# esrice/trio_binning

Hardware: AMD Instinct MI355X
Metric: Gbases/sec classified (k=21, 2x300M k-mer tables) (higher is better)
Workload: dtype u64

## Files before the change

include/tbk.h:

```cpp
#ifndef TBK_H
#define TBK_H

#include <stddef.h>
#include <stdint.h>

#ifdef __cplusplus
extern "C" {
#endif

#define TBK_ABI_VERSION 1

typedef enum tbk_status {
    TBK_OK = 0,
    TBK_ERR_INVALID = -1,
    TBK_ERR_IO = -2,
    TBK_ERR_FORMAT = -3,
    TBK_ERR_NO_DEVICE = -4,
    TBK_ERR_HIP = -5,
    TBK_ERR_NOMEM = -6,
    TBK_ERR_STATE = -7
} tbk_status;

typedef struct tbk_table tbk_table;
typedef struct tbk_classifier tbk_classifier;
// ... 39 lines not shown
    int32_t short_keys, entries, wide_entries, front;
    int32_t mod_sampling;
    int32_t span3;
    int32_t guests;
    int32_t minimizer_w;
    int32_t minimizer_m;
    int32_t two_read_kernel;
    double table_load;
    double entry_load, wentry_load, short_load;
    double clustered, behind_front, plainly_clustered, entry_min_ratio;
    uint64_t memory_budget_bytes;
    uint64_t table_align;
    uint32_t short_line_cap;
    int32_t probe_max_blocks;
    int32_t packed_h2d;
    uint64_t slice_bases;
    int32_t build_timing;
    int32_t force_replica;
    int32_t ring_streams, copy_priority, h2d_streams, zero_copy;
    int32_t full_keys;
    double full_load;
    int32_t replica_copy;
    int32_t verify_build;
} tbk_options;
void tbk_options_init(tbk_options *o);
int tbk_options_from_env(tbk_options *o);
int tbk_classifier_create_opts(const tbk_table *hap_a, const tbk_table *hap_b, const tbk_options *options, tbk_classifier **out);
int tbk_classifier_create_multi(const tbk_table *hap_a, const tbk_table *hap_b, const int *devices, int n_devices,
                                tbk_classifier **out );
int tbk_classifier_create_multi_opts(const tbk_table *hap_a, const tbk_table *hap_b, const int *devices, int n_devices,
                                     const tbk_options *options, tbk_classifier **out );
int tbk_classifier_replicate(const tbk_classifier *src, int device, tbk_classifier **out);
int tbk_classifier_table_id(const tbk_classifier *c, uint64_t *table_id, int *is_replica);
int tbk_classifier_device(const tbk_classifier *c);
int tbk_classifier_stats(const tbk_classifier *c, uint64_t *distinct_a, uint64_t *distinct_b,
                         uint64_t *n_buckets, uint64_t *table_bytes);
int tbk_classifier_shared_keys(const tbk_classifier *c, uint64_t *n_shared);
int tbk_classifier_layout(const tbk_classifier *c, int *minimizer_w, int *minimizer_m, int *span_offset);
int tbk_classifier_sampling_t(const tbk_classifier *c);
int tbk_classifier_build_info(const tbk_classifier *c, int *layout_builds, uint64_t *keys_past_half);
int tbk_classifier_front(const tbk_classifier *c, int *front, uint64_t *keys_behind_front);
int tbk_classifier_entries(const tbk_classifier *c, int *entry_layout, uint64_t *entries_a, uint64_t *entries_b);
int tbk_classifier_calibrate(tbk_classifier *c, double *lines_per_sec);
int tbk_classifier_calibrate_pairs(tbk_classifier *c, int inflight, int waves_per_simd, uint64_t n_lines, double *lines_per_sec);

int tbk_classify_batch(tbk_classifier *c, const uint8_t *bases, const uint64_t *offsets,
// ... 161 lines not shown
```

trio_binning_amd/_lib.py:

```python
import ctypes as C
import os

_HERE = os.path.dirname(os.path.abspath(__file__))
_NAME = "libtbk_hip.so"

TBK_OK = 0
TBK_ERR_INVALID = -1
TBK_ERR_IO = -2
TBK_ERR_FORMAT = -3
TBK_ERR_NO_DEVICE = -4
TBK_ERR_HIP = -5
TBK_ERR_NOMEM = -6
TBK_ERR_STATE = -7


class TbkError(RuntimeError):
    def __init__(self, code, message):
        super().__init__(f"libtbk_hip: {message} (status {code})")
        self.code = code
        self.message = message


def _find():
    override = os.environ.get("TBK_LIBRARY")
# ... 172 lines not shown
        _sig("tbk_fastx_inflates_on_device", C.c_int, _vp)
    if hasattr(lib, "tbk_bgzf_inflate_device"):
        _sig("tbk_bgzf_inflate_device", C.c_int, C.c_int, C.c_char_p, _u64, C.c_char_p, _u64, _u64p)
    if hasattr(lib, "tbk_bgzf_bench_device"):
        _sig("tbk_bgzf_bench_device", C.c_int, C.c_int, C.c_char_p, _u64, C.c_int, C.POINTER(C.c_double), C.POINTER(C.c_double), _u64p)
    if hasattr(lib, "tbk_gzip_bench_device"):
        _sig("tbk_gzip_bench_device", C.c_int, C.c_int, _vp, _u64p, _u64, C.c_int, C.POINTER(C.c_double), C.POINTER(C.c_double), _u64p)
_sig("tbk_gzip_member", C.c_int, C.c_char_p, C.c_size_t, C.c_char_p, C.c_size_t, C.POINTER(C.c_size_t))
_sig("tbk_crc32_c", C.c_uint32, C.c_uint32, C.c_char_p, C.c_size_t)
_sig("tbk_format_tsv", C.c_int, _vp, C.c_char_p, _vp, _vp, _vp, C.c_size_t, C.POINTER(C.c_size_t))
_sig("tbk_format_float", C.c_int, C.c_double, C.c_char_p, C.c_size_t)


class tbk_options(C.Structure):
    _fields_ = [("size", C.c_uint32),
                ("short_keys", C.c_int32), ("entries", C.c_int32), ("wide_entries", C.c_int32), ("front", C.c_int32),
                ("mod_sampling", C.c_int32), ("span3", C.c_int32), ("guests", C.c_int32), ("minimizer_w", C.c_int32), ("minimizer_m", C.c_int32),
                ("two_read_kernel", C.c_int32),
                ("table_load", C.c_double), ("entry_load", C.c_double), ("wentry_load", C.c_double), ("short_load", C.c_double),
                ("clustered", C.c_double), ("behind_front", C.c_double), ("plainly_clustered", C.c_double), ("entry_min_ratio", C.c_double),
                ("memory_budget_bytes", C.c_uint64), ("table_align", C.c_uint64), ("short_line_cap", C.c_uint32), ("probe_max_blocks", C.c_int32),
                ("packed_h2d", C.c_int32), ("slice_bases", C.c_uint64), ("build_timing", C.c_int32), ("force_replica", C.c_int32),
                ("ring_streams", C.c_int32), ("copy_priority", C.c_int32), ("h2d_streams", C.c_int32), ("zero_copy", C.c_int32),
                ("full_keys", C.c_int32), ("full_load", C.c_double), ("replica_copy", C.c_int32), ("verify_build", C.c_int32)]


HAS_OPTIONS = hasattr(lib, "tbk_classifier_create_opts")
if HAS_OPTIONS:
    _sig("tbk_options_init", None, C.POINTER(tbk_options))
    _sig("tbk_options_from_env", C.c_int, C.POINTER(tbk_options))
    _sig("tbk_classifier_create_opts", C.c_int, _vp, _vp, C.POINTER(tbk_options), C.POINTER(_vp))
    _sig("tbk_classifier_create_multi_opts", C.c_int, _vp, _vp, C.POINTER(C.c_int), C.c_int, C.POINTER(tbk_options), C.POINTER(_vp))
    _sig("tbk_pipeline_create_opts", C.c_int, _vp, _vp, C.POINTER(C.c_int), C.c_int, C.POINTER(tbk_options), C.POINTER(_vp))


def last_error() -> str:
    msg = lib.tbk_last_error()
    return msg.decode("utf-8", "replace") if msg else ""


def check(status: int) -> None:
    if status == TBK_OK:
        return
    msg = last_error()
    if status == TBK_ERR_IO:
        raise IOError(msg)
    if status in (TBK_ERR_FORMAT, TBK_ERR_INVALID):
# ... 45 lines not shown
```

trio_binning_amd/csrc/tbk_common.h:

```cpp
#pragma once
#include <stdint.h>
#include "tbk_tmer_order.h"

#ifdef __HIPCC__
#define TBK_HD __host__ __device__ __forceinline__
#else
#define TBK_HD inline
#endif

#define TBK_EMPTY 0xFFFFFFFFFFFFFFFFull
#define TBK_NOKEY 0xFFFFFFFFFFFFFFFEull
#define TBK_SLOTS_PER_BUCKET 8
#define TBK_BUCKET_BYTES 64
#define TBK_GUEST 0x8000000000000000ull

struct TbkMz {
    int w;
    int m;
    int o;
    int t;
};

TBK_HD uint32_t tbk_mix32(uint64_t key) {
    uint32_t lo = (uint32_t)key, hi = (uint32_t)(key >> 32);
    uint32_t h = lo * 0x9E3779B1u ^ (hi + 0x7F4A7C15u) * 0x85EBCA77u;
    h ^= h >> 15;
    h *= 0xC2B2AE3Du;
    h ^= h >> 13;
    return h;
}

TBK_HD uint32_t tbk_reduce(uint32_t h, uint32_t n_buckets) {
    return (uint32_t)(((uint64_t)h * (uint64_t)n_buckets) >> 32);
}
// ... 548 lines not shown
```

trio_binning_amd/csrc/tbk_host.cpp:

```cpp
#include <hip/hip_runtime.h>

#include <fcntl.h>
#include <sys/mman.h>
#include <sys/stat.h>
#include <unistd.h>

#include <algorithm>
#include <chrono>
#include <cmath>
#include <cerrno>
#include <cstdarg>
#include <cstdio>
#include <cstdlib>
#include <cstring>
#include <cctype>
#include <pthread.h>
#include <sched.h>
#include <atomic>
#include <memory>
#include <mutex>
#include <string>
#include <thread>
#include <vector>

#include "../../include/tbk.h"
#include "tbk_common.h"
#include "tbk_pack.h"

extern "C" hipError_t tbk_launch_order(uint64_t *, uint64_t, const uint32_t *, const uint32_t *, uint32_t, uint32_t, hipStream_t);
extern "C" hipError_t tbk_launch_insert(uint64_t *, uint32_t, uint32_t, uint32_t, TbkMz, const uint64_t *, uint64_t, uint32_t *, uint32_t *, uint32_t, TbkTableView,
                                        unsigned long long *, unsigned long long *, int *, hipStream_t);
extern "C" hipError_t tbk_launch_contains(TbkTableView, const uint64_t *, uint64_t, uint8_t *, hipStream_t);
extern "C" hipError_t tbk_launch_entry_insert(uint64_t *, uint32_t, uint32_t, TbkMz, int, const uint64_t *, uint64_t, int, int, unsigned long long *, int *, hipStream_t);
extern "C" hipError_t tbk_launch_short_insert(uint64_t *, uint32_t, uint32_t, uint32_t, TbkMz, int, const uint64_t *, uint64_t, int, unsigned long long *, int *, uint32_t, hipStream_t);
extern "C" hipError_t tbk_launch_full_insert(uint64_t *, uint32_t, uint32_t, TbkMz, int, const uint64_t *, uint64_t, int, unsigned long long *, int *, uint32_t, hipStream_t);
extern "C" hipError_t tbk_launch_probe_index(const uint64_t *, uint64_t, uint64_t, int32_t *, uint32_t *, uint64_t, int, hipStream_t);
extern "C" int tbk_probe_has_two_read_kernel(TbkMz);
extern "C" hipError_t tbk_launch_probe_range(const uint8_t *, const uint32_t *, const uint16_t *, const uint64_t *, uint64_t, uint64_t, TbkPairView, int,
                                             int32_t *, uint32_t *, uint64_t, uint64_t, uint64_t, int, int, hipEvent_t, hipStream_t, int);
extern "C" hipError_t tbk_launch_scatter_bad(const uint32_t *, const uint16_t *, uint64_t, uint16_t *, uint64_t, int, hipStream_t);
extern "C" uint64_t tbk_packed_chunks(uint64_t total_bases);
extern "C" uint64_t tbk_probe_passes(uint64_t total);
static constexpr uint64_t TBK_PASS_BASES = 2048;
extern "C" hipError_t tbk_launch_synth_keys(uint64_t, uint64_t, uint64_t, int, uint64_t *, hipStream_t);
extern "C" hipError_t tbk_launch_synth_reads(uint64_t, uint64_t, uint64_t, uint32_t, uint64_t, uint64_t, uint64_t,
                                             int, int, int, uint8_t *, uint64_t *, hipStream_t);
extern "C" hipError_t tbk_launch_fill(void *, uint64_t, uint64_t, hipStream_t);
extern "C" hipError_t tbk_launch_stream(const void *, uint64_t, uint32_t *, hipStream_t);
extern "C" hipError_t tbk_launch_gather(const void *, uint64_t, int, int, int, uint64_t, uint64_t, uint32_t *,
                                        uint64_t *, hipStream_t);

static thread_local std::string g_err;

static int fail(int code, const char *fmt, ...) {
    char buf[512];
    va_list ap;
    va_start(ap, fmt);
    vsnprintf(buf, sizeof buf, fmt, ap);
    va_end(ap);
    g_err = buf;
    return code;
}
// ... 27 lines not shown
    return end == v ? dflt : d;
}

extern "C" void tbk_options_init(tbk_options *o) {
    if (!o) return;
    memset(o, 0, sizeof *o);
    o->size = (uint32_t)sizeof *o;
    o->short_keys = o->entries = o->wide_entries = o->front = -1;
    o->full_keys = -1;
    o->full_load = 2.0;
    o->mod_sampling = o->span3 = o->guests = -1;
    o->minimizer_w = -1;
    o->minimizer_m = 0;
    o->two_read_kernel = 1;
    o->table_load = 0.0;
    o->entry_load = 0.5; o->wentry_load = 0.25; o->short_load = 2.3;
    o->clustered = 0.003; o->behind_front = 0.05; o->plainly_clustered = 0.12; o->entry_min_ratio = 1.5;
    o->memory_budget_bytes = 0;
    o->short_line_cap = 32;
    o->packed_h2d = 1;
    o->slice_bases = (uint64_t)384 << 20;
    o->h2d_streams = 1;
    o->verify_build = -1;
}

extern "C" int tbk_options_from_env(tbk_options *o) {
    if (!o) return fail(TBK_ERR_INVALID, "options is NULL");
    if (o->size != sizeof *o) tbk_options_init(o);
    auto tri = [](const char *name, int32_t &v) { const double d = env_double(name, -1); if (getenv(name) && *getenv(name)) v = d > 0 ? 1 : d == 0 ? 0 : -1; };
    auto num = [](const char *name, double &v) { if (getenv(name) && *getenv(name)) v = env_double(name, v); };
    auto inum = [](const char *name, int32_t &v) { if (getenv(name) && *getenv(name)) v = (int32_t)env_double(name, v); };
    auto unum = [](const char *name, uint64_t &v) { if (getenv(name) && *getenv(name)) v = (uint64_t)std::max(0.0, env_double(name, (double)v)); };
    tri("TBK_SHORT", o->short_keys); tri("TBK_ENTRY", o->entries); tri("TBK_ENTRY_WIDE", o->wide_entries); tri("TBK_FRONT", o->front);
    tri("TBK_FULL", o->full_keys); num("TBK_FULL_LOAD", o->full_load);
    tri("TBK_MOD_SAMPLING", o->mod_sampling); tri("TBK_SPAN3", o->span3); tri("TBK_GUESTS", o->guests);
    inum("TBK_MINIMIZER_W", o->minimizer_w); inum("TBK_MINIMIZER_M", o->minimizer_m); inum("TBK_TWO_READ", o->two_read_kernel);
    num("TBK_TABLE_LOAD", o->table_load); num("TBK_ENTRY_LOAD", o->entry_load); num("TBK_WENTRY_LOAD", o->wentry_load); num("TBK_SHORT_LOAD", o->short_load);
    num("TBK_CLUSTERED", o->clustered); num("TBK_BEHIND_FRONT", o->behind_front); num("TBK_PLAINLY_CLUSTERED", o->plainly_clustered);
    num("TBK_ENTRY_MIN_RATIO", o->entry_min_ratio);
    unum("TBK_MEMORY_BUDGET", o->memory_budget_bytes); unum("TBK_TABLE_ALIGN", o->table_align); unum("TBK_SLICE_BASES", o->slice_bases);
    { uint64_t cap = o->short_line_cap; unum("TBK_SHORT_LINE_CAP", cap); o->short_line_cap = (uint32_t)cap; }
    inum("TBK_PROBE_MAX_BLOCKS", o->probe_max_blocks); inum("TBK_PACKED_H2D", o->packed_h2d); inum("TBK_BUILD_TIMING", o->build_timing);
    inum("TBK_FORCE_REPLICA", o->force_replica); inum("TBK_RING_STREAMS", o->ring_streams); inum("TBK_COPY_PRIORITY", o->copy_priority);
    inum("TBK_H2D_STREAMS", o->h2d_streams); inum("TBK_ZERO_COPY", o->zero_copy);
    inum("TBK_REPLICA_COPY", o->replica_copy); tri("TBK_VERIFY_BUILD", o->verify_build);
    return TBK_OK;
}

static tbk_options resolve_options(const tbk_options *in) {
    tbk_options o;
    tbk_options_init(&o);
    if (in && in->size >= 8) memcpy(&o, in, std::min<size_t>(in->size, sizeof o));
    o.size = (uint32_t)sizeof o;
    return o;
}

static long local_ranks() {
    long ranks = (long)env_double("TBK_LOCAL_RANKS", 0);
    if (ranks < 1) ranks = (long)env_double("LOCAL_WORLD_SIZE", 1);
    return std::max<long>(1, ranks);
}

static long usable_cpus() {
    long n = (long)std::thread::hardware_concurrency();
    if (n < 1) n = 1;
    cpu_set_t set;
    if (sched_getaffinity(0, sizeof set, &set) == 0 && CPU_COUNT(&set) > 0) n = std::min<long>(n, CPU_COUNT(&set));
// ... 1733 lines not shown
    }
    delete c;
}

static void par_memcpy(void *dst, const void *src, size_t n) {
    const size_t piece = (size_t)16 << 20;
    const int nt = (int)std::min<size_t>((size_t)tbk_host_threads(), n / piece);
    if (nt <= 1) { memcpy(dst, src, n); return; }
    std::vector<std::thread> pool;
    for (int t = 0; t < nt; t++) {
        const size_t lo = n * (size_t)t / nt, hi = n * (size_t)(t + 1) / nt;
        pool.emplace_back([=]() { memcpy((char *)dst + lo, (const char *)src + lo, hi - lo); });
    }
    for (std::thread &th : pool) th.join();
}

static bool is_pinned(const void *p) {
    hipPointerAttribute_t at;
    hipError_t e = hipPointerGetAttributes(&at, p);
    if (e != hipSuccess) { (void)hipGetLastError(); return false; }
    return at.type == hipMemoryTypeHost;
}

struct ProbeSlice { uint64_t pass_lo, pass_hi; hipEvent_t arrived; };

static int launch_probe_timed(tbk_classifier *c, const uint8_t *d_bases, const uint64_t *d_offsets,
                              uint64_t n_reads, uint64_t total, int32_t *d_counts, const uint32_t *d_codes = nullptr,
                              const uint16_t *d_bad16 = nullptr, const ProbeSlice *slices = nullptr, int n_slices = 0) {
    if (n_reads >= 0xFFFFFFF0ull) return fail(TBK_ERR_INVALID, "more than 2^32 reads in one batch");
    if (total == 0) {
        HIP_TRY(hipMemsetAsync(d_counts, 0, n_reads * 2 * sizeof(int32_t), c->compute));
        return TBK_OK;
    }
    const uint64_t passes = tbk_probe_passes(total);
    if (passes > c->cap_passes) {
        HIP_TRY(hipStreamSynchronize(c->compute));
        if (c->d_pass_read) HIP_TRY(hipFree(c->d_pass_read));
        c->d_pass_read = nullptr; c->cap_passes = 0;
        const uint64_t cap = (passes + passes / 4 + 1024 + 1) & ~1ull;
        HIP_TRY(hipMalloc((void **)&c->d_pass_read, (4 * cap + 16) * sizeof(uint32_t)));
        c->cap_passes = cap;
    }
    const ProbeSlice whole = {0, passes, nullptr};
    if (n_slices <= 0) { slices = &whole; n_slices = 1; }
    hipEvent_t *ev = nullptr;
    if (c->timing) {
        const size_t need = 2 + 3 * (size_t)n_slices;
        if (c->ev_used + need > c->ev.size() && c->ev.size() >= (size_t)TIMING_POOL) {
            HIP_TRY(hipStreamSynchronize(c->compute));
            int rc = c->fold_timing();
            if (rc) return rc;
        }
        while (c->ev_used + need > c->ev.size()) {
            hipEvent_t a;
            HIP_TRY(hipEventCreate(&a));
            c->ev.push_back(a);
        }
        ev = c->ev.data() + c->ev_used;
        c->ev_used += need;
        c->ev_slices.push_back((uint32_t)n_slices);
        c->timed_launches++;
        HIP_TRY(hipEventRecord(ev[0], c->compute));
    }
    HIP_TRY(tbk_launch_probe_index(d_offsets, n_reads, total, d_counts, c->d_pass_read, c->cap_passes, c->opt.two_read_kernel != 0 && tbk_probe_has_two_read_kernel(c->mz), c->compute));
    if (ev) HIP_TRY(hipEventRecord(ev[1], c->compute));
    for (int j = 0; j < n_slices; j++) {
        if (slices[j].arrived) HIP_TRY(hipStreamWaitEvent(c->compute, slices[j].arrived, 0));
        if (ev) HIP_TRY(hipEventRecord(ev[2 + 3 * j], c->compute));
        HIP_TRY(tbk_launch_probe_range(d_bases, d_codes, d_bad16, d_offsets, n_reads, total, c->pair(), c->k, d_counts, c->d_pass_read, c->cap_passes,
                                       slices[j].pass_lo, slices[j].pass_hi, c->max_blocks, c->opt.two_read_kernel != 0, ev ? ev[3 + 3 * j] : nullptr, c->compute, 0));
        if (ev) HIP_TRY(hipEventRecord(ev[4 + 3 * j], c->compute));
    }
    c->last_passes = passes;
    return TBK_OK;
}

int tbk_classifier::fold_timing() {
    size_t at = 0;
    for (uint32_t n_slices : ev_slices) {
        float ms = 0;
        HIP_TRY(hipEventElapsedTime(&ms, ev[at], ev[at + 1]));
        timed_ms += ms;
        for (uint32_t j = 0; j < n_slices; j++) {
            float whole = 0, single = 0;
            HIP_TRY(hipEventElapsedTime(&whole, ev[at + 2 + 3 * j], ev[at + 4 + 3 * j]));
            HIP_TRY(hipEventElapsedTime(&single, ev[at + 3 + 3 * j], ev[at + 4 + 3 * j]));
            timed_ms += whole;
            timed_single_ms += single;
        }
        at += 2 + 3 * (size_t)n_slices;
    }
    ev_used = 0;
    ev_slices.clear();
// ... 149 lines not shown
        rc = slot_reserve_packed(s, n_chunks, n_exc);
        if (rc) return rc;
    }
    s.ticket = tk; s.n_reads = n_reads; s.user_counts = counts; s.counts_staged = !out_pinned;
    if (n_reads && total) {
        const uint64_t *src_o = offsets;
        if (!offs_pinned) { memcpy(s.h_offsets, offsets, (n_reads + 1) * sizeof(uint64_t)); src_o = s.h_offsets; }
        const uint8_t *src_b = bases;
        if (!packed && !bases_pinned) { par_memcpy(s.h_bases, bases, total); src_b = s.h_bases; }
        std::lock_guard<std::mutex> together(c->streams->enqueue);
        HIP_TRY(hipMemcpyAsync(s.d_offsets, src_o, (n_reads + 1) * sizeof(uint64_t), hipMemcpyHostToDevice, c->copy));
        if (packed) {
            if (!s.bad_clean) HIP_TRY(hipMemsetAsync(s.d_bad, 0, (s.cap_chunks + 2) * sizeof(uint16_t), c->copy));
            s.bad_clean = false;
            if (n_exc) {
                HIP_TRY(hipMemcpyAsync(s.d_exc_chunk, exc_chunk, n_exc * sizeof(uint32_t), hipMemcpyHostToDevice, c->copy));
                HIP_TRY(hipMemcpyAsync(s.d_exc_mask, exc_mask, n_exc * sizeof(uint16_t), hipMemcpyHostToDevice, c->copy));
            }
        }
        HIP_TRY(hipEventRecord(s.copied, c->copy));
        const uint64_t passes = tbk_probe_passes(total);
        const bool zero_copy = packed && c->opt.zero_copy != 0 && is_pinned(codes);
        const bool alone = c->streams->in_flight.load() == 0;
        const int n_slices = alone ? (int)std::max<uint64_t>(1, std::min<uint64_t>(8, total / c->slice_bases)) : 1;
        ProbeSlice slices[8];
        uint64_t sent = 0;
        for (int j = 0; j < n_slices; j++) {
            slices[j].pass_lo = passes * (uint64_t)j / (uint64_t)n_slices;
            slices[j].pass_hi = passes * (uint64_t)(j + 1) / (uint64_t)n_slices;
            slices[j].arrived = s.sliced[j];
            const uint64_t upto = j + 1 == n_slices ? n_chunks : std::min<uint64_t>(n_chunks, slices[j].pass_hi * (TBK_PASS_BASES / 16) + 2);
            if (upto > sent) {
                if (packed && zero_copy) {
                } else if (packed && n_slices == 1 && c->streams->copy2 && upto - sent >= ((uint64_t)1 << 22)) {
                    const uint64_t mid = sent + (upto - sent) / 2;
                    HIP_TRY(hipMemcpyAsync(s.d_codes + mid, codes + mid, (upto - mid) * sizeof(uint32_t), hipMemcpyHostToDevice, c->streams->copy2));
                    HIP_TRY(hipEventRecord(s.copied2, c->streams->copy2));
                    HIP_TRY(hipMemcpyAsync(s.d_codes + sent, codes + sent, (mid - sent) * sizeof(uint32_t), hipMemcpyHostToDevice, c->copy));
                    HIP_TRY(hipStreamWaitEvent(c->copy, s.copied2, 0));
                } else if (packed) {
                    HIP_TRY(hipMemcpyAsync(s.d_codes + sent, codes + sent, (upto - sent) * sizeof(uint32_t), hipMemcpyHostToDevice, c->copy));
                } else {
                    const uint64_t b0 = sent * 16, b1 = std::min<uint64_t>(total, upto * 16);
                    HIP_TRY(hipMemcpyAsync(s.d_bases + b0, src_b + b0, b1 - b0, hipMemcpyHostToDevice, c->copy));
                }
                sent = upto;
            }
            HIP_TRY(hipEventRecord(s.sliced[j], c->copy));
        }
        HIP_TRY(hipStreamWaitEvent(c->compute, s.copied, 0));
        if (packed) HIP_TRY(tbk_launch_scatter_bad(s.d_exc_chunk, s.d_exc_mask, n_exc, s.d_bad, total, 0, c->compute));
        rc = launch_probe_timed(c, packed ? nullptr : s.d_bases, s.d_offsets, n_reads, total, s.d_counts, packed ? (zero_copy ? const_cast<uint32_t *>(codes) : s.d_codes) : nullptr,
                                packed ? s.d_bad : nullptr, slices, n_slices);
        if (rc) return rc;
// ... 200 lines not shown
}

extern "C" int tbk_kernel_timing_read2(tbk_classifier *c, uint64_t *launches, double *total_ms, double *single_ms) {
    if (!c || !launches || !total_ms) return fail(TBK_ERR_INVALID, "NULL argument");
    int rc = use_device(c->device);
    if (rc) return rc;
    HIP_TRY(hipStreamSynchronize(c->compute));
    rc = c->fold_timing();
    if (rc) return rc;
    *launches = c->timed_launches;
    *total_ms = c->timed_ms;
    if (single_ms) *single_ms = c->timed_single_ms;
    c->timed_launches = 0; c->timed_ms = 0.0; c->timed_single_ms = 0.0;
    return TBK_OK;
}

extern "C" int tbk_classifier_last_passes(tbk_classifier *c, uint64_t *n_passes, uint64_t *n_multi) {
    if (!c || !n_passes || !n_multi) return fail(TBK_ERR_INVALID, "NULL argument");
    *n_passes = c->last_passes; *n_multi = 0;
    if (!c->last_passes || !c->d_pass_read) return TBK_OK;
    int rc = use_device(c->device);
    if (rc) return rc;
    HIP_TRY(hipStreamSynchronize(c->compute));
    uint32_t m[2] = {0, 0};
    HIP_TRY(hipMemcpy(m, c->d_pass_read + 4 * c->cap_passes, sizeof m, hipMemcpyDeviceToHost));
    *n_multi = (uint64_t)m[0] + m[1];
    return TBK_OK;
}

extern "C" int tbk_kernel_timing_read(tbk_classifier *c, uint64_t *launches, double *total_ms) {
    return tbk_kernel_timing_read2(c, launches, total_ms, nullptr);
}

static std::mutex g_cache_mu;
static tbk_classifier *g_cached = nullptr;
static const tbk_table *g_cached_a = nullptr, *g_cached_b = nullptr;

static void drop_cached_classifier(const tbk_table *t) {
    std::lock_guard<std::mutex> lk(g_cache_mu);
    if (g_cached && (g_cached_a == t || g_cached_b == t)) {
        tbk_classifier_destroy(g_cached);
        g_cached = nullptr; g_cached_a = g_cached_b = nullptr;
    }
}

static constexpr uint64_t SMALL_READ_MAX = (uint64_t)8 << 20;

static int count_small(tbk_classifier *c, const char *read, uint64_t len, int *count_a, int *count_b) {
    int rc = use_device(c->device);
    if (rc) return rc;
    if (len > c->small_cap) {
        c->small_free();
        const uint64_t cap = std::max<uint64_t>((uint64_t)1 << 20, len + len / 2);
        const uint64_t pass_cap = (tbk_probe_passes(cap) + 2) & ~1ull;
        hipError_t e = hipHostMalloc((void **)&c->small_h, 64 + cap + 4096, hipHostMallocPortable | hipHostMallocMapped);
        if (e == hipSuccess) e = hipHostMalloc((void **)&c->small_h_counts, 64, hipHostMallocPortable);
        if (e == hipSuccess) e = hipMalloc((void **)&c->small_d_counts, 64);
        if (e == hipSuccess) e = hipMemset(c->small_d_counts, 0, 64);
        if (e == hipSuccess) e = hipMalloc((void **)&c->small_scratch, (4 * pass_cap + 16) * sizeof(uint32_t));
        if (e == hipSuccess) e = hipMemset(c->small_scratch, 0, (4 * pass_cap + 16) * sizeof(uint32_t));
        if (e == hipSuccess) e = hipDeviceSynchronize();
        if (e != hipSuccess) { (void)hipGetLastError(); c->small_free(); return TBK_ERR_STATE; }
        memset(c->small_h, 0, 64 + cap + 4096);
        c->small_cap = cap; c->small_pass_cap = pass_cap;
        c->small_last[0] = c->small_last[1] = 0;
    }
    uint64_t *offsets = (uint64_t *)c->small_h;
    uint8_t *bases = c->small_h + 64;
    offsets[0] = 0; offsets[1] = len;
    memcpy(bases, read, len);
    std::lock_guard<std::mutex> together(c->streams->enqueue);
    hipError_t e = tbk_launch_probe_range(bases, nullptr, nullptr, offsets, 1, len, c->pair(), c->k, c->small_d_counts, c->small_scratch, c->small_pass_cap, 0,
                                          tbk_probe_passes(len), c->max_blocks, 0, nullptr, c->compute, 1);
    if (e == hipSuccess) e = hipMemcpyAsync(c->small_h_counts, c->small_d_counts, 2 * sizeof(int32_t), hipMemcpyDeviceToHost, c->compute);
    if (e == hipSuccess) e = hipStreamSynchronize(c->compute);
    if (e != hipSuccess) {
        c->small_free();
        return fail(TBK_ERR_HIP, "tbk_count_kmers_in_read: %s", hipGetErrorString(e));
    }
    const uint32_t now_a = c->small_h_counts[0], now_b = c->small_h_counts[1];
    *count_a = (int)(uint32_t)(now_a - c->small_last[0]);
    *count_b = (int)(uint32_t)(now_b - c->small_last[1]);
    c->small_last[0] = now_a; c->small_last[1] = now_b;
    return TBK_OK;
}

extern "C" int tbk_count_kmers_in_read(const char *read, int64_t len, const tbk_table *a, const tbk_table *b,
                                       int *count_a, int *count_b) {
    if (!read || !a || !b || !count_a || !count_b) return fail(TBK_ERR_INVALID, "NULL argument");
    if (len < 0) len = (int64_t)strlen(read);
    std::lock_guard<std::mutex> lk(g_cache_mu);
    if (!g_cached || g_cached_a != a || g_cached_b != b) {
        if (g_cached) { tbk_classifier_destroy(g_cached); g_cached = nullptr; }
        int rc = tbk_classifier_create(a, b, &g_cached);
        if (rc) return rc;
        g_cached_a = a; g_cached_b = b;
// ... 322 lines not shown
```

trio_binning_amd/csrc/tbk_kernels.hip:

```cpp
#include <hip/hip_runtime.h>
#include <stdint.h>

#include <algorithm>
#include <type_traits>

#include "tbk_common.h"
#include "tbk_device.h"

__device__ __forceinline__ bool tbk_lookup_slow(const TbkTableView t, uint64_t key) {
    if (key >= TBK_NOKEY) return false;
    uint32_t b = tbk_bucket_of(key, t.mz, t.n_buckets);
    for (uint32_t walked = 0; walked <= t.n_buckets; walked++) {
        const uint64_t *line = t.slots + (uint64_t)b * t.stride;
        for (uint32_t s = 0; s < TBK_SLOTS_PER_BUCKET; s++)
            if (line[tbk_slot_at(t.guests, t.stride, t.half, s)] == key) return true;
        if (t.stride == 16 && (t.guests & (TBK_FLAG_FRONT | TBK_FLAG_GUESTS)) == (TBK_FLAG_FRONT | TBK_FLAG_GUESTS))
            for (uint32_t s = 0; s < 4; s++)
                if (line[tbk_slot_at(t.guests, t.stride, t.half ^ 8u, s)] == (key | TBK_GUEST)) return true;
        if (!(line[tbk_slot_at(t.guests, t.stride, t.half, 6)] > line[tbk_slot_at(t.guests, t.stride, t.half, 7)])) return false;
        if (t.guests & TBK_FLAG_GUESTS) {
            for (uint32_t s = 0; s < TBK_SLOTS_PER_BUCKET; s++)
                if (line[tbk_slot_at(t.guests, t.stride, t.half ^ 8u, s)] == (key | TBK_GUEST)) return true;
            if (!(line[tbk_slot_at(t.guests, t.stride, t.half, 4)] > line[tbk_slot_at(t.guests, t.stride, t.half, 5)])) return false;
        }
// ... 1620 lines not shown
        const uint32_t ca = rcnt[2 * lane], cb = rcnt[2 * lane + 1];
        if (ca) { atomicAdd(&p.counts[2 * (r_first + lane)], (int)ca); rcnt[2 * lane] = 0; }
        if (cb) { atomicAdd(&p.counts[2 * (r_first + lane) + 1], (int)cb); rcnt[2 * lane + 1] = 0; }
        __builtin_amdgcn_fence(__ATOMIC_ACQ_REL, "wavefront");
    }
    if (TWO) {
        __builtin_amdgcn_fence(__ATOMIC_ACQ_REL, "wavefront");
        if (lane < 4) {
            const uint32_t c = rcnt[lane] + (lane == 0 ? acc_a : lane == 1 ? acc_b : lane == 2 ? acc2_a : acc2_b);
            if (c) atomicAdd(&p.counts[2 * r_first + lane], (int)c);
            rcnt[lane] = 0;
        }
        __builtin_amdgcn_fence(__ATOMIC_ACQ_REL, "wavefront");
    } else if (!MULTI) {
        if (lane == 0) {
            if (acc_a) atomicAdd(&p.counts[2 * r_first], (int)acc_a);
            if (acc_b) atomicAdd(&p.counts[2 * r_first + 1], (int)acc_b);
        }
    }
}

__global__ void __launch_bounds__(1024)
tbk_pass_index_kernel(const uint64_t *__restrict__ offsets, uint64_t n_reads, uint64_t total, uint64_t n_passes,
                      uint32_t *__restrict__ pass_read, uint32_t *__restrict__ multi_list, uint32_t *__restrict__ n_multi,
                      uint64_t *__restrict__ two_list, uint32_t *__restrict__ n_two, int use_two, int32_t *__restrict__ counts) {
    const uint64_t pass = (uint64_t)blockIdx.x * blockDim.x + threadIdx.x;
    bool to_multi = false, to_two = false;
    uint32_t r_first_of_pass = 0;
    if (pass < n_passes) {
        const uint64_t P0 = pass * TBK_PASS;
        const uint64_t r_first = find_read(offsets, n_reads, P0);
        pass_read[pass] = (uint32_t)r_first;
        r_first_of_pass = (uint32_t)r_first;
        const uint64_t last_pos = P0 + TBK_PASS - 1 < total ? P0 + TBK_PASS - 1 : total - 1;
        const uint64_t r_end = r_first < n_reads ? offsets[r_first + 1] : total;
        if (last_pos >= r_end) {
            to_two = use_two && r_end > P0 && offsets[r_first + 2] > last_pos;
            to_multi = !to_two;
        }
    }
    __shared__ uint32_t s_count[2], s_base[2];
    if (threadIdx.x < 2) s_count[threadIdx.x] = 0;
    __syncthreads();
    const uint32_t lane = threadIdx.x & 63u;
    uint32_t in_wave[2] = {0, 0}, wave_at[2] = {0, 0};
    const bool mine[2] = {to_multi, to_two};
#pragma unroll
    for (int l = 0; l < 2; l++) {
        const uint64_t m = __builtin_amdgcn_ballot_w64(mine[l]);
        if (m != 0) {
            const int leader = __builtin_ctzll(m);
            uint32_t base = 0;
            if ((int)lane == leader) base = atomicAdd(&s_count[l], (uint32_t)__popcll(m));
            wave_at[l] = (uint32_t)__shfl((int)base, leader, 64);
            in_wave[l] = (uint32_t)__popcll(m & ((1ull << lane) - 1ull));
        }
    }
    __syncthreads();
    if (threadIdx.x < 2 && s_count[threadIdx.x] != 0) s_base[threadIdx.x] = atomicAdd(threadIdx.x == 0 ? n_multi : n_two, s_count[threadIdx.x]);
    __syncthreads();
    if (to_multi) multi_list[s_base[0] + wave_at[0] + in_wave[0]] = (uint32_t)pass;
    if (to_two) two_list[s_base[1] + wave_at[1] + in_wave[1]] = pass | ((uint64_t)r_first_of_pass << 32);
    const uint64_t step = (uint64_t)gridDim.x * blockDim.x;
    for (uint64_t i = pass; i < 2 * n_reads; i += step) counts[i] = 0;
}

template <int W, bool M64, bool SAMP, bool FRONT, bool MULTI, bool TWO = false>
__global__ void __launch_bounds__(64 * TBK_WAVES_PER_BLOCK, MULTI ? TBK_MIN_WAVES_MULTI
                                                               : TWO ? (FRONT && W <= 7 ? TBK_MIN_WAVES : 4)
                                                               : (FRONT ? TBK_MIN_WAVES : (W <= 6 ? TBK_MIN_WAVES_WHOLE : 4)))
tbk_probe_kernel(const ProbeArgs p) {
    __shared__ uint64_t stage[TBK_WAVES_PER_BLOCK][TBK_CHUNKS + 2];
    __shared__ uint4 walkq[TBK_WAVES_PER_BLOCK][FRONT ? TBK_QCAP_FRONT : TBK_QCAP];
    __shared__ uint4 backq[TBK_WAVES_PER_BLOCK][FRONT ? TBK_BQCAP : 1];
    __shared__ uint32_t rcnt[TBK_WAVES_PER_BLOCK][MULTI ? 2 * TBK_RCNT : (TWO ? 4 : 1)];
    const uint32_t lane = threadIdx.x & 63u;
#if TBK_OCC_PAD
    __shared__ uint32_t occ_pad[TBK_OCC_PAD / 4];
    occ_pad[threadIdx.x] = 0;
    if (p.k == 99) p.counts[0] = (int32_t)occ_pad[(threadIdx.x * 97u) % (TBK_OCC_PAD / 4)];
#endif
    const uint32_t wave = (uint32_t)__builtin_amdgcn_readfirstlane((int)(threadIdx.x >> 6));
    const uint64_t per_iter = (uint64_t)gridDim.x * TBK_WAVES_PER_BLOCK;
    if (MULTI) { rcnt[wave][lane] = 0; rcnt[wave][64 + lane] = 0; }
    if (TWO && lane < 4) rcnt[wave][lane] = 0;
// ... 164 lines not shown
    }
}

extern "C" hipError_t tbk_launch_scatter_bad(const uint32_t *d_exc_chunk, const uint16_t *d_exc_mask, uint64_t n, uint16_t *d_bad16,
                                             uint64_t total, int clear, hipStream_t stream) {
    if (n == 0 && (total & 15u) == 0) return hipSuccess;
    hipLaunchKernelGGL(tbk_scatter_bad_kernel, dim3((unsigned)((std::max<uint64_t>(n, 1) + 255) / 256)), dim3(256), 0, stream, d_exc_chunk, d_exc_mask, n, d_bad16, total, clear);
    return hipGetLastError();
}

static void fill_args(ProbeArgs &p, const uint8_t *d_bases, const uint32_t *d_codes, const uint16_t *d_bad16, const uint64_t *d_offsets,
                      uint64_t n_reads, uint64_t total, TbkPairView t, int k, int32_t *d_counts, uint32_t *d_scratch, uint64_t pass_cap) {
    p.codes = d_codes; p.bad16 = d_bad16; p.n_chunks = (total + 15) / 16;
    p.bases = d_bases; p.offsets = d_offsets; p.n_reads = n_reads; p.total = total;
    p.n_passes = (total + TBK_PASS - 1) / TBK_PASS;
    p.t = t; p.k = k; p.counts = d_counts; p.pass_read = d_scratch; p.multi_list = d_scratch + pass_cap; p.two_list = (const uint64_t *)(d_scratch + 2 * pass_cap);
    p.n_multi = d_scratch + 4 * pass_cap; p.n_two = d_scratch + 4 * pass_cap + 1;
    p.pass_lo = 0; p.pass_hi = p.n_passes;
}

extern "C" int tbk_probe_has_two_read_kernel(TbkMz mz) { return mz.w >= 2 && mz.t > 0; }

extern "C" hipError_t tbk_launch_probe_index(const uint64_t *d_offsets, uint64_t n_reads, uint64_t total, int32_t *d_counts, uint32_t *d_scratch,
                                             uint64_t pass_cap, int use_two, hipStream_t stream) {
    if (total == 0 || n_reads == 0) return hipSuccess;
    const uint64_t n_passes = (total + TBK_PASS - 1) / TBK_PASS;
    if (n_passes > pass_cap) return hipErrorInvalidValue;
    uint32_t *d_multi = d_scratch + pass_cap, *d_n = d_scratch + 4 * pass_cap;
    uint64_t *d_two = (uint64_t *)(d_scratch + 2 * pass_cap);
    if (pass_cap & 1) return hipErrorInvalidValue;
    hipError_t e = hipMemsetAsync(d_n, 0, 2 * sizeof(uint32_t), stream);
    if (e != hipSuccess) return e;
    hipLaunchKernelGGL(tbk_pass_index_kernel, dim3((unsigned)((n_passes + 1023) / 1024)), dim3(1024), 0, stream,
                       d_offsets, n_reads, total, n_passes, d_scratch, d_multi, d_n, d_two, d_n + 1, use_two, d_counts);
    return hipGetLastError();
}

extern "C" hipError_t tbk_launch_probe_range(const uint8_t *d_bases, const uint32_t *d_codes, const uint16_t *d_bad16, const uint64_t *d_offsets,
                                             uint64_t n_reads, uint64_t total, TbkPairView t, int k, int32_t *d_counts, uint32_t *d_scratch,
                                             uint64_t pass_cap, uint64_t pass_lo, uint64_t pass_hi, int max_blocks, int use_two, hipEvent_t between, hipStream_t stream,
                                             int only_single) {
    if (total == 0 || n_reads == 0 || pass_hi <= pass_lo) return hipSuccess;
    ProbeArgs p;
    fill_args(p, d_bases, d_codes, d_bad16, d_offsets, n_reads, total, t, k, d_counts, d_scratch, pass_cap);
    if (p.n_passes > pass_cap || pass_hi > p.n_passes) return hipErrorInvalidValue;
    p.pass_lo = pass_lo; p.pass_hi = pass_hi;
    const uint64_t blocks = (pass_hi - pass_lo + TBK_WAVES_PER_BLOCK - 1) / TBK_WAVES_PER_BLOCK;
    uint64_t blocks_multi = std::min<uint64_t>(blocks, 16384);
    if (max_blocks > 0 && blocks_multi > (uint64_t)max_blocks) blocks_multi = (uint64_t)max_blocks;
    const dim3 grid((unsigned)blocks), grid_multi((unsigned)blocks_multi), block(64 * TBK_WAVES_PER_BLOCK);
    const bool m64 = t.mz.m > 16, samp = t.mz.t > 0, front = (t.guests & TBK_FLAG_FRONT) != 0, entry = (t.guests & TBK_FLAG_ENTRY) != 0;
    if (front && t.mz.w < 2) return hipErrorInvalidValue;
    const bool wide = (t.guests & TBK_FLAG_WIDE) != 0, shortk = (t.guests & TBK_FLAG_SHORT) != 0, fullk = (t.guests & TBK_FLAG_FULL) != 0;
    const bool span3 = (entry || shortk) && t.mz.t > 0 && t.mz.t == t.mz.m - 2 * t.mz.w;
    if ((entry || shortk) && t.mz.t > 0 && !span3 && t.mz.t != t.mz.m - t.mz.w) return hipErrorInvalidValue;
    if (TBK_TMER_LUT && span3 && t.mz.w == 6 && t.mz.t != 4) return hipErrorInvalidValue;
    if (shortk) {
        TbkShortGeom g;
        if (!tbk_short_geom(k, t.mz, t.n_buckets, &g) || t.n_buckets > 0x3FFFFFFFu) return hipErrorInvalidValue;
    }
    if (fullk && (!tbk_full_geom(k, t.mz) || t.mz.t != t.mz.m - t.mz.w || t.n_buckets > 0x3FFFFFFFu)) return hipErrorInvalidValue;
    if (entry) {
        TbkEntryGeom g;
        if (!(wide ? tbk_wentry_geom(k, t.mz, &g) : tbk_entry_geom(k, t.mz, &g)) || t.n_buckets > 0x3FFFFFFFu) return hipErrorInvalidValue;
    }
    const uint64_t blocks_two = use_two && tbk_probe_has_two_read_kernel(t.mz) ? std::min<uint64_t>(n_reads > 1 ? n_reads - 1 : 0, p.n_passes) : 0;
    const dim3 grid_two((unsigned)std::max<uint64_t>(1, blocks_two));
    hipError_t e = hipSuccess;
    for (int which = 2; which >= 0; which--) {
        if (which == 1 && blocks_two == 0) continue;
        if (which != 0 && only_single) continue;
        if (which == 0 && between != nullptr) { e = hipEventRecord(between, stream); if (e != hipSuccess) return e; }
#define TBK_LAUNCH(N, M, S, F) do { if (which == 2) hipLaunchKernelGGL((tbk_probe_kernel<N, M, S, F, true>), grid_multi, block, 0, stream, p); \
                                    else if (which == 0) hipLaunchKernelGGL((tbk_probe_kernel<N, M, S, F, false>), grid, block, 0, stream, p); \
                                    else if (S && N >= 2) hipLaunchKernelGGL((tbk_probe_kernel<N, M, (S && N >= 2), F, false, (S && N >= 2)>), grid_two, block, 0, stream, p); } while (0)
#define TBK_W(N) case N: if (samp && front) { if (m64) TBK_LAUNCH(N, true, true, true); else TBK_LAUNCH(N, false, true, true); } \
                         else if (samp) { if (m64) TBK_LAUNCH(N, true, true, false); else TBK_LAUNCH(N, false, true, false); } \
                         else if (front) { if (m64) TBK_LAUNCH(N, true, false, true); else TBK_LAUNCH(N, false, false, true); } \
                         else { if (m64) TBK_LAUNCH(N, true, false, false); else TBK_LAUNCH(N, false, false, false); } break;
        if (entry || shortk || fullk) {
#define TBK_E1(N, WD, LW) do { if (which == 2) hipLaunchKernelGGL((tbk_probe_entry_kernel<N, true, false, WD, LW>), grid_multi, block, 0, stream, p); \
                         else if (which == 0) hipLaunchKernelGGL((tbk_probe_entry_kernel<N, false, false, WD, LW>), grid, block, 0, stream, p); \
                         else hipLaunchKernelGGL((tbk_probe_entry_kernel<N, false, true, WD, LW>), grid_two, block, 0, stream, p); } while (0)
#define TBK_E(N, WD) case N: if (span3) TBK_E1(N, WD, 3); else TBK_E1(N, WD, 2); break;
#define TBK_E2(N, WD) case N: if (span3) return hipErrorInvalidValue; TBK_E1(N, WD, 2); break;
            if (fullk) {
                switch (t.mz.w) {
#ifdef TBK_ONLY_W6
                    TBK_E2(6, 3) TBK_E2(8, 3)
// ... 71 lines not shown
```

Measured before the change: 224.4.

## Partition probe multi/two-read worklists per slice and allow steady-state slicing

The pass index kernel now builds separate multi-pass and two-read worklists per slice, each with its own counter, so each sliced probe launch handles only its own slice's entries. The two-read kernel grid is sized from the slice's pass range and the number of read boundaries that fall inside it. A new steady_slices option allows slicing when other batches are in flight, but it defaults to 1, so the steady path is unchanged by default. The intent is to cut redundant work and oversized grids in the sliced probes that overlap copies, at the cost of per-slice loops and extra syncs in the index kernel plus host binary searches.

```diff
diff --git a/include/tbk.h b/include/tbk.h
--- a/include/tbk.h
+++ b/include/tbk.h
@@ -85,6 +85,7 @@
     double full_load;
     int32_t replica_copy;
     int32_t verify_build;
+    int32_t steady_slices;
 } tbk_options;
 void tbk_options_init(tbk_options *o);
 int tbk_options_from_env(tbk_options *o);
diff --git a/trio_binning_amd/_lib.py b/trio_binning_amd/_lib.py
--- a/trio_binning_amd/_lib.py
+++ b/trio_binning_amd/_lib.py
@@ -218,7 +218,8 @@
                 ("memory_budget_bytes", C.c_uint64), ("table_align", C.c_uint64), ("short_line_cap", C.c_uint32), ("probe_max_blocks", C.c_int32),
                 ("packed_h2d", C.c_int32), ("slice_bases", C.c_uint64), ("build_timing", C.c_int32), ("force_replica", C.c_int32),
                 ("ring_streams", C.c_int32), ("copy_priority", C.c_int32), ("h2d_streams", C.c_int32), ("zero_copy", C.c_int32),
-                ("full_keys", C.c_int32), ("full_load", C.c_double), ("replica_copy", C.c_int32), ("verify_build", C.c_int32)]
+                ("full_keys", C.c_int32), ("full_load", C.c_double), ("replica_copy", C.c_int32), ("verify_build", C.c_int32),
+                ("steady_slices", C.c_int32)]
 
 
 HAS_OPTIONS = hasattr(lib, "tbk_classifier_create_opts")
diff --git a/trio_binning_amd/csrc/tbk_common.h b/trio_binning_amd/csrc/tbk_common.h
--- a/trio_binning_amd/csrc/tbk_common.h
+++ b/trio_binning_amd/csrc/tbk_common.h
@@ -10,6 +10,9 @@
 
 #define TBK_EMPTY 0xFFFFFFFFFFFFFFFFull
 #define TBK_NOKEY 0xFFFFFFFFFFFFFFFEull
+#define TBK_MAX_SLICES 8
+TBK_HD uint64_t tbk_slice_lo(uint64_t passes, uint32_t j, uint32_t n_slices) { return passes * j / n_slices; }
+TBK_HD uint32_t tbk_slice_of(uint64_t pass, uint64_t passes, uint32_t n_slices) { return (uint32_t)(((pass + 1) * n_slices - 1) / passes); }
 #define TBK_SLOTS_PER_BUCKET 8
 #define TBK_BUCKET_BYTES 64
 #define TBK_GUEST 0x8000000000000000ull
diff --git a/trio_binning_amd/csrc/tbk_host.cpp b/trio_binning_amd/csrc/tbk_host.cpp
--- a/trio_binning_amd/csrc/tbk_host.cpp
+++ b/trio_binning_amd/csrc/tbk_host.cpp
@@ -34,10 +34,10 @@
 extern "C" hipError_t tbk_launch_entry_insert(uint64_t *, uint32_t, uint32_t, TbkMz, int, const uint64_t *, uint64_t, int, int, unsigned long long *, int *, hipStream_t);
 extern "C" hipError_t tbk_launch_short_insert(uint64_t *, uint32_t, uint32_t, uint32_t, TbkMz, int, const uint64_t *, uint64_t, int, unsigned long long *, int *, uint32_t, hipStream_t);
 extern "C" hipError_t tbk_launch_full_insert(uint64_t *, uint32_t, uint32_t, TbkMz, int, const uint64_t *, uint64_t, int, unsigned long long *, int *, uint32_t, hipStream_t);
-extern "C" hipError_t tbk_launch_probe_index(const uint64_t *, uint64_t, uint64_t, int32_t *, uint32_t *, uint64_t, int, hipStream_t);
+extern "C" hipError_t tbk_launch_probe_index(const uint64_t *, uint64_t, uint64_t, int32_t *, uint32_t *, uint64_t, int, int, hipStream_t);
 extern "C" int tbk_probe_has_two_read_kernel(TbkMz);
 extern "C" hipError_t tbk_launch_probe_range(const uint8_t *, const uint32_t *, const uint16_t *, const uint64_t *, uint64_t, uint64_t, TbkPairView, int,
-                                             int32_t *, uint32_t *, uint64_t, uint64_t, uint64_t, int, int, hipEvent_t, hipStream_t, int);
+                                             int32_t *, uint32_t *, uint64_t, int, int, uint64_t, int, int, hipEvent_t, hipStream_t, int);
 extern "C" hipError_t tbk_launch_scatter_bad(const uint32_t *, const uint16_t *, uint64_t, uint16_t *, uint64_t, int, hipStream_t);
 extern "C" uint64_t tbk_packed_chunks(uint64_t total_bases);
 extern "C" uint64_t tbk_probe_passes(uint64_t total);
@@ -111,6 +111,7 @@
     o->slice_bases = (uint64_t)384 << 20;
     o->h2d_streams = 1;
     o->verify_build = -1;
+    o->steady_slices = 1;
 }
 
 extern "C" int tbk_options_from_env(tbk_options *o) {
@@ -132,6 +133,7 @@
     inum("TBK_PROBE_MAX_BLOCKS", o->probe_max_blocks); inum("TBK_PACKED_H2D", o->packed_h2d); inum("TBK_BUILD_TIMING", o->build_timing);
     inum("TBK_FORCE_REPLICA", o->force_replica); inum("TBK_RING_STREAMS", o->ring_streams); inum("TBK_COPY_PRIORITY", o->copy_priority);
     inum("TBK_H2D_STREAMS", o->h2d_streams); inum("TBK_ZERO_COPY", o->zero_copy);
+    inum("TBK_STEADY_SLICES", o->steady_slices);
     inum("TBK_REPLICA_COPY", o->replica_copy); tri("TBK_VERIFY_BUILD", o->verify_build);
     return TBK_OK;
 }
@@ -1911,7 +1913,7 @@
     return at.type == hipMemoryTypeHost;
 }
 
-struct ProbeSlice { uint64_t pass_lo, pass_hi; hipEvent_t arrived; };
+struct ProbeSlice { hipEvent_t arrived; uint64_t read_ends; };
 
 static int launch_probe_timed(tbk_classifier *c, const uint8_t *d_bases, const uint64_t *d_offsets,
                               uint64_t n_reads, uint64_t total, int32_t *d_counts, const uint32_t *d_codes = nullptr,
@@ -1930,7 +1932,7 @@
         HIP_TRY(hipMalloc((void **)&c->d_pass_read, (4 * cap + 16) * sizeof(uint32_t)));
         c->cap_passes = cap;
     }
-    const ProbeSlice whole = {0, passes, nullptr};
+    const ProbeSlice whole = {nullptr, 0};
     if (n_slices <= 0) { slices = &whole; n_slices = 1; }
     hipEvent_t *ev = nullptr;
     if (c->timing) {
@@ -1951,13 +1953,13 @@
         c->timed_launches++;
         HIP_TRY(hipEventRecord(ev[0], c->compute));
     }
-    HIP_TRY(tbk_launch_probe_index(d_offsets, n_reads, total, d_counts, c->d_pass_read, c->cap_passes, c->opt.two_read_kernel != 0 && tbk_probe_has_two_read_kernel(c->mz), c->compute));
+    HIP_TRY(tbk_launch_probe_index(d_offsets, n_reads, total, d_counts, c->d_pass_read, c->cap_passes, c->opt.two_read_kernel != 0 && tbk_probe_has_two_read_kernel(c->mz), n_slices, c->compute));
     if (ev) HIP_TRY(hipEventRecord(ev[1], c->compute));
     for (int j = 0; j < n_slices; j++) {
         if (slices[j].arrived) HIP_TRY(hipStreamWaitEvent(c->compute, slices[j].arrived, 0));
         if (ev) HIP_TRY(hipEventRecord(ev[2 + 3 * j], c->compute));
         HIP_TRY(tbk_launch_probe_range(d_bases, d_codes, d_bad16, d_offsets, n_reads, total, c->pair(), c->k, d_counts, c->d_pass_read, c->cap_passes,
-                                       slices[j].pass_lo, slices[j].pass_hi, c->max_blocks, c->opt.two_read_kernel != 0, ev ? ev[3 + 3 * j] : nullptr, c->compute, 0));
+                                       j, n_slices, slices[j].read_ends, c->max_blocks, c->opt.two_read_kernel != 0, ev ? ev[3 + 3 * j] : nullptr, c->compute, 0));
         if (ev) HIP_TRY(hipEventRecord(ev[4 + 3 * j], c->compute));
     }
     c->last_passes = passes;
@@ -2153,14 +2155,16 @@
         const uint64_t passes = tbk_probe_passes(total);
         const bool zero_copy = packed && c->opt.zero_copy != 0 && is_pinned(codes);
         const bool alone = c->streams->in_flight.load() == 0;
-        const int n_slices = alone ? (int)std::max<uint64_t>(1, std::min<uint64_t>(8, total / c->slice_bases)) : 1;
-        ProbeSlice slices[8];
+        const uint64_t most = alone ? TBK_MAX_SLICES : (uint64_t)std::min(TBK_MAX_SLICES, std::max(1, (int)c->opt.steady_slices));
+        const int n_slices = (int)std::max<uint64_t>(1, std::min<uint64_t>(most, total / c->slice_bases));
+        ProbeSlice slices[TBK_MAX_SLICES];
         uint64_t sent = 0;
         for (int j = 0; j < n_slices; j++) {
-            slices[j].pass_lo = passes * (uint64_t)j / (uint64_t)n_slices;
-            slices[j].pass_hi = passes * (uint64_t)(j + 1) / (uint64_t)n_slices;
+            const uint64_t pass_lo = tbk_slice_lo(passes, (uint32_t)j, (uint32_t)n_slices), pass_hi = tbk_slice_lo(passes, (uint32_t)j + 1, (uint32_t)n_slices);
             slices[j].arrived = s.sliced[j];
-            const uint64_t upto = j + 1 == n_slices ? n_chunks : std::min<uint64_t>(n_chunks, slices[j].pass_hi * (TBK_PASS_BASES / 16) + 2);
+            slices[j].read_ends = std::max<uint64_t>(1, (uint64_t)(std::lower_bound(offsets + 1, offsets + n_reads + 1, pass_hi * TBK_PASS_BASES) -
+                                                                   std::upper_bound(offsets + 1, offsets + n_reads + 1, pass_lo * TBK_PASS_BASES)));
+            const uint64_t upto = j + 1 == n_slices ? n_chunks : std::min<uint64_t>(n_chunks, pass_hi * (TBK_PASS_BASES / 16) + 2);
             if (upto > sent) {
                 if (packed && zero_copy) {
                 } else if (packed && n_slices == 1 && c->streams->copy2 && upto - sent >= ((uint64_t)1 << 22)) {
@@ -2407,9 +2411,9 @@
     int rc = use_device(c->device);
     if (rc) return rc;
     HIP_TRY(hipStreamSynchronize(c->compute));
-    uint32_t m[2] = {0, 0};
+    uint32_t m[2 * TBK_MAX_SLICES];
     HIP_TRY(hipMemcpy(m, c->d_pass_read + 4 * c->cap_passes, sizeof m, hipMemcpyDeviceToHost));
-    *n_multi = (uint64_t)m[0] + m[1];
+    for (uint32_t listed : m) *n_multi += listed;
     return TBK_OK;
 }
 
@@ -2456,7 +2460,7 @@
     memcpy(bases, read, len);
     std::lock_guard<std::mutex> together(c->streams->enqueue);
     hipError_t e = tbk_launch_probe_range(bases, nullptr, nullptr, offsets, 1, len, c->pair(), c->k, c->small_d_counts, c->small_scratch, c->small_pass_cap, 0,
-                                          tbk_probe_passes(len), c->max_blocks, 0, nullptr, c->compute, 1);
+                                          1, 0, c->max_blocks, 0, nullptr, c->compute, 1);
     if (e == hipSuccess) e = hipMemcpyAsync(c->small_h_counts, c->small_d_counts, 2 * sizeof(int32_t), hipMemcpyDeviceToHost, c->compute);
     if (e == hipSuccess) e = hipStreamSynchronize(c->compute);
     if (e != hipSuccess) {
diff --git a/trio_binning_amd/csrc/tbk_kernels.hip b/trio_binning_amd/csrc/tbk_kernels.hip
--- a/trio_binning_amd/csrc/tbk_kernels.hip
+++ b/trio_binning_amd/csrc/tbk_kernels.hip
@@ -1666,8 +1666,8 @@
 
 __global__ void __launch_bounds__(1024)
 tbk_pass_index_kernel(const uint64_t *__restrict__ offsets, uint64_t n_reads, uint64_t total, uint64_t n_passes,
-                      uint32_t *__restrict__ pass_read, uint32_t *__restrict__ multi_list, uint32_t *__restrict__ n_multi,
-                      uint64_t *__restrict__ two_list, uint32_t *__restrict__ n_two, int use_two, int32_t *__restrict__ counts) {
+                      uint32_t *__restrict__ pass_read, uint32_t *__restrict__ multi_list, uint64_t *__restrict__ two_list,
+                      uint32_t *__restrict__ n_lists, uint32_t n_slices, int use_two, int32_t *__restrict__ counts) {
     const uint64_t pass = (uint64_t)blockIdx.x * blockDim.x + threadIdx.x;
     bool to_multi = false, to_two = false;
     uint32_t r_first_of_pass = 0;
@@ -1684,27 +1684,36 @@
         }
     }
     __shared__ uint32_t s_count[2], s_base[2];
-    if (threadIdx.x < 2) s_count[threadIdx.x] = 0;
-    __syncthreads();
     const uint32_t lane = threadIdx.x & 63u;
-    uint32_t in_wave[2] = {0, 0}, wave_at[2] = {0, 0};
-    const bool mine[2] = {to_multi, to_two};
-#pragma unroll
-    for (int l = 0; l < 2; l++) {
-        const uint64_t m = __builtin_amdgcn_ballot_w64(mine[l]);
-        if (m != 0) {
-            const int leader = __builtin_ctzll(m);
-            uint32_t base = 0;
-            if ((int)lane == leader) base = atomicAdd(&s_count[l], (uint32_t)__popcll(m));
-            wave_at[l] = (uint32_t)__shfl((int)base, leader, 64);
-            in_wave[l] = (uint32_t)__popcll(m & ((1ull << lane) - 1ull));
-        }
-    }
-    __syncthreads();
-    if (threadIdx.x < 2 && s_count[threadIdx.x] != 0) s_base[threadIdx.x] = atomicAdd(threadIdx.x == 0 ? n_multi : n_two, s_count[threadIdx.x]);
-    __syncthreads();
-    if (to_multi) multi_list[s_base[0] + wave_at[0] + in_wave[0]] = (uint32_t)pass;
-    if (to_two) two_list[s_base[1] + wave_at[1] + in_wave[1]] = pass | ((uint64_t)r_first_of_pass << 32);
+    const uint64_t block_first = (uint64_t)blockIdx.x * blockDim.x;
+    const uint64_t block_last = block_first + blockDim.x - 1 < n_passes ? block_first + blockDim.x - 1 : n_passes - 1;
+    const uint32_t j_lo = n_slices > 1 ? tbk_slice_of(block_first, n_passes, n_slices) : 0;
+    const uint32_t j_hi = n_slices > 1 ? tbk_slice_of(block_last, n_passes, n_slices) : 0;
+    const uint32_t my_slice = n_slices > 1 && pass < n_passes ? tbk_slice_of(pass, n_passes, n_slices) : 0;
+    for (uint32_t j = j_lo; j <= j_hi; j++) {
+        if (threadIdx.x < 2) s_count[threadIdx.x] = 0;
+        __syncthreads();
+        const bool here = my_slice == j;
+        uint32_t in_wave[2] = {0, 0}, wave_at[2] = {0, 0};
+        const bool mine[2] = {to_multi && here, to_two && here};
+#pragma unroll
+        for (int l = 0; l < 2; l++) {
+            const uint64_t m = __builtin_amdgcn_ballot_w64(mine[l]);
+            if (m != 0) {
+                const int leader = __builtin_ctzll(m);
+                uint32_t base = 0;
+                if ((int)lane == leader) base = atomicAdd(&s_count[l], (uint32_t)__popcll(m));
+                wave_at[l] = (uint32_t)__shfl((int)base, leader, 64);
+                in_wave[l] = (uint32_t)__popcll(m & ((1ull << lane) - 1ull));
+            }
+        }
+        __syncthreads();
+        if (threadIdx.x < 2 && s_count[threadIdx.x] != 0) s_base[threadIdx.x] = atomicAdd(&n_lists[2 * j + threadIdx.x], s_count[threadIdx.x]);
+        __syncthreads();
+        const uint64_t at = tbk_slice_lo(n_passes, j, n_slices);
+        if (mine[0]) multi_list[at + s_base[0] + wave_at[0] + in_wave[0]] = (uint32_t)pass;
+        if (mine[1]) two_list[at + s_base[1] + wave_at[1] + in_wave[1]] = pass | ((uint64_t)r_first_of_pass << 32);
+    }
     const uint64_t step = (uint64_t)gridDim.x * blockDim.x;
     for (uint64_t i = pass; i < 2 * n_reads; i += step) counts[i] = 0;
 }
@@ -1915,29 +1924,34 @@
 extern "C" int tbk_probe_has_two_read_kernel(TbkMz mz) { return mz.w >= 2 && mz.t > 0; }
 
 extern "C" hipError_t tbk_launch_probe_index(const uint64_t *d_offsets, uint64_t n_reads, uint64_t total, int32_t *d_counts, uint32_t *d_scratch,
-                                             uint64_t pass_cap, int use_two, hipStream_t stream) {
+                                             uint64_t pass_cap, int use_two, int n_slices, hipStream_t stream) {
     if (total == 0 || n_reads == 0) return hipSuccess;
+    if (n_slices < 1 || n_slices > TBK_MAX_SLICES) return hipErrorInvalidValue;
     const uint64_t n_passes = (total + TBK_PASS - 1) / TBK_PASS;
     if (n_passes > pass_cap) return hipErrorInvalidValue;
     uint32_t *d_multi = d_scratch + pass_cap, *d_n = d_scratch + 4 * pass_cap;
     uint64_t *d_two = (uint64_t *)(d_scratch + 2 * pass_cap);
     if (pass_cap & 1) return hipErrorInvalidValue;
-    hipError_t e = hipMemsetAsync(d_n, 0, 2 * sizeof(uint32_t), stream);
+    hipError_t e = hipMemsetAsync(d_n, 0, 2 * TBK_MAX_SLICES * sizeof(uint32_t), stream);
     if (e != hipSuccess) return e;
     hipLaunchKernelGGL(tbk_pass_index_kernel, dim3((unsigned)((n_passes + 1023) / 1024)), dim3(1024), 0, stream,
-                       d_offsets, n_reads, total, n_passes, d_scratch, d_multi, d_n, d_two, d_n + 1, use_two, d_counts);
+                       d_offsets, n_reads, total, n_passes, d_scratch, d_multi, d_two, d_n, (uint32_t)n_slices, use_two, d_counts);
     return hipGetLastError();
 }
 
 extern "C" hipError_t tbk_launch_probe_range(const uint8_t *d_bases, const uint32_t *d_codes, const uint16_t *d_bad16, const uint64_t *d_offsets,
                                              uint64_t n_reads, uint64_t total, TbkPairView t, int k, int32_t *d_counts, uint32_t *d_scratch,
-                                             uint64_t pass_cap, uint64_t pass_lo, uint64_t pass_hi, int max_blocks, int use_two, hipEvent_t between, hipStream_t stream,
-                                             int only_single) {
-    if (total == 0 || n_reads == 0 || pass_hi <= pass_lo) return hipSuccess;
+                                             uint64_t pass_cap, int slice, int n_slices, uint64_t two_cap, int max_blocks, int use_two, hipEvent_t between,
+                                             hipStream_t stream, int only_single) {
+    if (total == 0 || n_reads == 0) return hipSuccess;
+    if (n_slices < 1 || n_slices > TBK_MAX_SLICES || slice < 0 || slice >= n_slices) return hipErrorInvalidValue;
     ProbeArgs p;
     fill_args(p, d_bases, d_codes, d_bad16, d_offsets, n_reads, total, t, k, d_counts, d_scratch, pass_cap);
-    if (p.n_passes > pass_cap || pass_hi > p.n_passes) return hipErrorInvalidValue;
+    if (p.n_passes > pass_cap) return hipErrorInvalidValue;
+    const uint64_t pass_lo = tbk_slice_lo(p.n_passes, (uint32_t)slice, (uint32_t)n_slices), pass_hi = tbk_slice_lo(p.n_passes, (uint32_t)slice + 1, (uint32_t)n_slices);
+    if (pass_hi <= pass_lo) return hipSuccess;
     p.pass_lo = pass_lo; p.pass_hi = pass_hi;
+    p.multi_list += pass_lo; p.two_list += pass_lo; p.n_multi += 2 * slice; p.n_two += 2 * slice;
     const uint64_t blocks = (pass_hi - pass_lo + TBK_WAVES_PER_BLOCK - 1) / TBK_WAVES_PER_BLOCK;
     uint64_t blocks_multi = std::min<uint64_t>(blocks, 16384);
     if (max_blocks > 0 && blocks_multi > (uint64_t)max_blocks) blocks_multi = (uint64_t)max_blocks;
@@ -1957,7 +1971,8 @@
         TbkEntryGeom g;
         if (!(wide ? tbk_wentry_geom(k, t.mz, &g) : tbk_entry_geom(k, t.mz, &g)) || t.n_buckets > 0x3FFFFFFFu) return hipErrorInvalidValue;
     }
-    const uint64_t blocks_two = use_two && tbk_probe_has_two_read_kernel(t.mz) ? std::min<uint64_t>(n_reads > 1 ? n_reads - 1 : 0, p.n_passes) : 0;
+    uint64_t blocks_two = use_two && tbk_probe_has_two_read_kernel(t.mz) ? std::min<uint64_t>(n_reads > 1 ? n_reads - 1 : 0, pass_hi - pass_lo) : 0;
+    if (two_cap > 0 && blocks_two > two_cap) blocks_two = two_cap;
     const dim3 grid_two((unsigned)std::max<uint64_t>(1, blocks_two));
     hipError_t e = hipSuccess;
     for (int which = 2; which >= 0; which--) {
```

Result: no change. 223.2 (-0.5%).
